# ModelCloud/GPTQModel

Hardware: NVIDIA H100
Metric: W4A16 g128 QuantLinear: decode tok/s + prefill TFLOPS vs HBM/TC roofline (higher is better)
Workload: dtype f16

## Files before the change

gptqmodel_b200/csrc/b2q_decode.cu:

```cuda
#include "b2q_common.cuh"
#include "b2q_decode.cuh"
#include "b2q_internal.h"

namespace b2q {

template <typename T, bool ASYM, bool G64, bool MOE>
__global__ void __launch_bounds__(DEC_MAX_WARPS * 32)
    decode_kernel(const __grid_constant__ DecSets S, const int32_t* __restrict__ perm, const T* __restrict__ x, int M,
                  int K, int gsh, int qpc, int max_tiles, int ngroups, int stl,
                  const __grid_constant__ DecodeAR ar, unsigned long long* __restrict__ trace) {
  using E = ET<T>;
  extern __shared__ __align__(128) uint8_t dsm[];
  auto stamp = [&](int slot) {
    if (trace != nullptr && threadIdx.x == 0 && blockIdx.y == 0) {
      unsigned long long tns;
      asm volatile("mov.u64 %0, %%globaltimer;" : "=l"(tns));
      trace[blockIdx.x * 16 + slot] = tns;
    }
  };
  stamp(0);
  if (MOE) asm volatile("griddepcontrol.wait;" ::: "memory");
  const int lane = threadIdx.x & 31, warp = threadIdx.x >> 5, nwarps = blockDim.x >> 5;
  const int g = lane >> 2, t = lane & 3;
  const int gw = nwarps / ngroups;
  const int grp = warp / gw, wg = warp - grp * gw;
  const int C = gridDim.x * ngroups;
  const int tile0 = (int)blockIdx.x * ngroups + grp;
  const int TT = S.tile_end[S.nsets - 1];
  const int ntiles = (tile0 < TT) ? (TT - tile0 + C - 1) / C : 0;
  const int nquads = K >> 7;
  const int q0 = (MOE && S.moe >= 2) ? 0 : blockIdx.y * qpc;
  const int q1 = min(q0 + qpc, nquads);
  const int kspan = qpc * 128;
  if (MOE && S.moe >= 2) x += (size_t)blockIdx.y * K * (S.moe == 3 ? 2 : 1);
  const int nst = 1 << stl;
  uint8_t* ring = dsm + (size_t)warp * nst * DEC_QUAD_BYTES;
  T* sx = reinterpret_cast<T*>(dsm + (size_t)nwarps * nst * DEC_QUAD_BYTES);
  float* xsum = reinterpret_cast<float*>(reinterpret_cast<uint8_t*>(sx) + (size_t)M * kspan * sizeof(T));
  float* red = xsum + qpc * 2 * 8;
  float* part = red + 2 * nwarps * 256;
  const uint32_t bars = smem_u32(part + max_tiles * 256) + warp * DEC_STAGES * 8;
  const bool PERM = perm != nullptr;

  const int nq = (q0 + wg < q1) ? (q1 - q0 - wg + gw - 1) / gw : 0;
  const int U = ntiles * nq;
  const uint4* iss_src = nullptr;
  size_t iss_kbs = 0;
  int iss_q = 0, iss_u = 0, iss_ti = 0;
  auto iss_begin_tile = [&]() {
    const TileRef<T> r = resolve_tile<T, MOE>(S, tile0 + iss_ti * C);
    iss_kbs = (size_t)(r.N >> 4) * 32;
    iss_src = r.w + (size_t)(2 * (q0 + wg)) * iss_kbs + (size_t)(2 * r.nt) * 32;
  };
  auto iss_one = [&](uint32_t dst, uint32_t bar) {
    issue_quad(dst, bar, iss_src, iss_kbs);
    ++iss_u;
    if (++iss_q == nq) {
      iss_q = 0;
      ++iss_ti;
      if (iss_u < U) iss_begin_tile();
    } else {
      iss_src += (size_t)(2 * gw) * iss_kbs;
    }
  };
  if (lane == 0) {
#pragma unroll
    for (int i = 0; i < DEC_STAGES; ++i) mbar_init(bars + 8 * i, 1);
    fence_mbar_init();
    if (U > 0) iss_begin_tile();
#pragma unroll
    for (int i = 0; i < DEC_STAGES; ++i)
      if (i < nst && iss_u < U) iss_one(smem_u32(ring) + i * DEC_QUAD_BYTES, bars + 8 * i);
  }
  const int gstep = (2 * gw) >> gsh;
  const int g_first = (2 * (q0 + wg)) >> gsh;
  const T* sc_next = nullptr;
  const uint32_t* zq_next = nullptr;
  int pre_q = 0, pre_ti = 0, pre_N = 0;
  auto pre_begin_tile = [&]() {
    const TileRef<T> r = resolve_tile<T, MOE>(S, tile0 + pre_ti * C);
    pre_N = r.N;
    sc_next = r.sc + (size_t)g_first * r.N + r.nt * 32 + g;
    if (ASYM) zq_next = r.zq + (size_t)g_first * (r.N >> 3) + r.nt * 4;
  };
  auto fetch_scales = [&](DScale<ASYM, G64>& d) {
#pragma unroll
    for (int i = 0; i < 4; ++i) {
      d.s[0][i] = *reinterpret_cast<const uint16_t*>(sc_next + i * 8);
      if (ASYM) d.zw[0][i] = zq_next[i];
    }
    if (G64) {
#pragma unroll
      for (int i = 0; i < 4; ++i) {
        d.s[G64 ? 1 : 0][i] = *reinterpret_cast<const uint16_t*>(sc_next + (size_t)pre_N + i * 8);
        if (ASYM) d.zw[G64 ? 1 : 0][i] = zq_next[(pre_N >> 3) + i];
      }
    }
    if (++pre_q == nq) {
      pre_q = 0;
      ++pre_ti;
      if (pre_ti < ntiles) pre_begin_tile();
    } else {
      sc_next += (size_t)gstep * pre_N;
      if (ASYM) zq_next += (size_t)gstep * (pre_N >> 3);
    }
  };
  DScale<ASYM, G64> cur;
  if (U > 0) {
    pre_begin_tile();
    fetch_scales(cur);
  }

  if (PERM) prefetch_inverse_perm(perm + K, K);
  const bool OWN = !PERM && ngroups == 1;
  if (OWN) {
    zero_own_xsum_padding(xsum, M, nq, wg, gw);
  } else {
    for (int i = threadIdx.x; i < (q1 - q0) * 2 * 8; i += blockDim.x)
      if ((i & 7) >= M) xsum[i] = 0.f;
  }
  stamp(1);
  asm volatile("griddepcontrol.launch_dependents;" ::: "memory");
  asm volatile("griddepcontrol.wait;" ::: "memory");
  stamp(2);

  if (MOE && S.moe == 3) {
    stage_x_own_quads<T, true>(x, sx, xsum, 1, K, q0, nq, wg, gw, kspan);
  } else if (OWN) {
    stage_x_own_quads<T>(x, sx, xsum, M, K, q0, nq, wg, gw, kspan);
  } else if (PERM) {
    stage_x_act_order<T>(x, perm + K, sx, xsum, M, K, q0 * 128, (q1 - q0) * 128, kspan);
  } else {
    const int n8 = (q1 - q0) * 16;
    const int tot = M * n8;
    const int totr = (tot + 31) & ~31;
    constexpr int SX_UNROLL = 4;
    auto f2 = [](uint32_t u) {
      const T* h = reinterpret_cast<const T*>(&u);
      return E::to_f(h[0]) + E::to_f(h[1]);
    };
    for (int i0 = threadIdx.x; i0 < totr; i0 += blockDim.x * SX_UNROLL) {
      uint4 xv[SX_UNROLL];
      int mm[SX_UNROLL], jj[SX_UNROLL];
#pragma unroll
      for (int u = 0; u < SX_UNROLL; ++u) {
        const int i = i0 + u * blockDim.x;
        xv[u] = make_uint4(0, 0, 0, 0);
        mm[u] = 0;
        jj[u] = 0;
        if (i < tot) {
          const int m = (M == 1) ? 0 : i / n8, j = i - m * n8;
          mm[u] = m;
          jj[u] = j;
          const T* xr = x + (size_t)m * K;
          xv[u] = reinterpret_cast<const uint4*>(xr + (size_t)q0 * 128)[j];
        }
      }
#pragma unroll
      for (int u = 0; u < SX_UNROLL; ++u) {
        const int i = i0 + u * blockDim.x;
        if (i < totr) {
          if (i < tot) reinterpret_cast<uint4*>(sx + (size_t)mm[u] * kspan)[jj[u]] = xv[u];
          float sm = (f2(xv[u].x) + f2(xv[u].y)) + (f2(xv[u].z) + f2(xv[u].w));
          sm += __shfl_xor_sync(0xffffffffu, sm, 1);
          sm += __shfl_xor_sync(0xffffffffu, sm, 2);
          sm += __shfl_xor_sync(0xffffffffu, sm, 4);
          if ((i & 7) == 0 && i < tot) xsum[(jj[u] >> 3) * 8 + mm[u]] = sm;
        }
      }
    }
  }
  if (!OWN) __syncthreads();
  stamp(3);

  constexpr float ZSYM = 8.f;
  const uint32_t nrank = cluster_nctarank();
  const uint32_t ring_a = smem_u32(ring) + lane * 16;
  const uint32_t xf_a0 = smem_u32(sx) + (uint32_t)((g * kspan + t * 16 + wg * 128) * 2);
  const uint32_t xs_a0 = smem_u32(xsum) + (uint32_t)((2 * t + wg * 16) * 4);
  const uint32_t xf_qstep = (uint32_t)gw * 256u, xs_qstep = (uint32_t)gw * 64u;
  uint32_t ar_seq = 0;
  if (ar.world > 1) ar_seq = *reinterpret_cast<const volatile uint32_t*>(ar.ctl);
  int u = 0;
  for (int ti = 0; ti < ntiles; ++ti) {
    const TileRef<T> tr = resolve_tile<T, MOE>(S, tile0 + ti * C);
    const int nt = tr.nt, N = tr.N;
    const T* bias = tr.bias;
    T* out = tr.out;
    float tot[2][4];
#pragma unroll
    for (int a = 0; a < 2; ++a)
#pragma unroll
      for (int b = 0; b < 4; ++b) tot[a][b] = 0.f;

    uint32_t xf_a = xf_a0, xs_a = xs_a0;
    for (int qi = 0; qi < nq; ++qi, ++u, xf_a += xf_qstep, xs_a += xs_qstep) {
      DScale<ASYM, G64> nxt;
      if (u + 1 < U) fetch_scales(nxt);
      const int st = u & (nst - 1);
      mbar_wait(bars + 8 * st, (uint32_t)(u >> stl) & 1u);
      const uint32_t wq_a = ring_a + st * DEC_QUAD_BYTES;
      float dd[2][2][4];
#pragma unroll
      for (int a = 0; a < 2; ++a)
#pragma unroll
        for (int b = 0; b < 2; ++b)
#pragma unroll
          for (int c = 0; c < 4; ++c) dd[a][b][c] = 0.f;
      float xs0 = 0.f, xs1 = 0.f;
#pragma unroll
      for (int kbl = 0; kbl < 2; ++kbl) {
        uint32_t bx[8];
        if (g < M) {
          const uint4 x0 = lds128(xf_a + kbl * 128), x1 = lds128(xf_a + kbl * 128 + 16);
          bx[0] = x0.x; bx[1] = x0.y; bx[2] = x0.z; bx[3] = x0.w;
          bx[4] = x1.x; bx[5] = x1.y; bx[6] = x1.z; bx[7] = x1.w;
        } else {
#pragma unroll
          for (int r = 0; r < 8; ++r) bx[r] = 0u;
        }
#pragma unroll
        for (int ftl = 0; ftl < 2; ++ftl) {
          const uint4 wv = lds128(wq_a + (kbl * 2 + ftl) * 512);
          const uint32_t w[4] = {wv.x, wv.y, wv.z, wv.w};
#pragma unroll
          for (int s = 0; s < 4; ++s) {
            uint32_t a[4];
            E::unpack_w4(w[s], a);
            mma_16816<T>(dd[kbl][ftl], a, bx[2 * s], bx[2 * s + 1]);
          }
        }
        const float2 xs = lds_f2(xs_a + kbl * 32);
        xs0 += xs.x;
        xs1 += xs.y;
        if (kbl == 1 || G64) {
          const int gi = G64 ? kbl : 0;
#pragma unroll
          for (int ftl = 0; ftl < 2; ++ftl) {
            const uint16_t slr = cur.s[gi][ftl * 2], shr = cur.s[gi][ftl * 2 + 1];
            const float sl = E::to_f(*reinterpret_cast<const T*>(&slr));
            const float sh = E::to_f(*reinterpret_cast<const T*>(&shr));
            float zl = ZSYM, zh = ZSYM;
            if (ASYM) {
              zl = (float)((cur.zw[ASYM ? gi : 0][ftl * 2] >> (4 * g)) & 15u);
              zh = (float)((cur.zw[ASYM ? gi : 0][ftl * 2 + 1] >> (4 * g)) & 15u);
            }
            const float bl = E::LO_BASE + zl, bh = E::HI_BASE + zh;
            float d[4];
#pragma unroll
            for (int c = 0; c < 4; ++c) d[c] = G64 ? dd[kbl][ftl][c] : dd[0][ftl][c] + dd[1][ftl][c];
            tot[ftl][0] = fmaf(sl, d[0] - bl * xs0, tot[ftl][0]);
            tot[ftl][1] = fmaf(sl, d[1] - bl * xs1, tot[ftl][1]);
            tot[ftl][2] = fmaf(sh, d[2] * E::HI_SCALE - bh * xs0, tot[ftl][2]);
            tot[ftl][3] = fmaf(sh, d[3] * E::HI_SCALE - bh * xs1, tot[ftl][3]);
          }
          xs0 = xs1 = 0.f;
        }
      }
      __syncwarp();
      if (lane == 0 && iss_u < U) iss_one(ring_a + st * DEC_QUAD_BYTES, bars + 8 * st);
      if (u + 1 < U) cur = nxt;
    }

    if (ti < 5) stamp(4 + 2 * ti);
    float* rbuf = red + (grp * 2 + (ti & 1)) * gw * 256;
#pragma unroll
    for (int a = 0; a < 2; ++a)
#pragma unroll
      for (int b = 0; b < 4; ++b) rbuf[(wg * 8 + a * 4 + b) * 32 + lane] = tot[a][b];
    asm volatile("bar.sync %0, %1;" ::"r"(1 + grp), "r"(gw * 32) : "memory");
    for (int i = wg * 32 + lane; i < 256; i += gw * 32) {
      float v = 0.f;
      for (int w = 0; w < gw; ++w) v += rbuf[w * 256 + i];
      if (nrank > 1) {
        part[(grp * max_tiles + ti) * 256 + i] = v;
      } else {
        const int acc = i >> 5, ln = i & 31;
        const int m = 2 * (ln & 3) + (acc & 1);
        if (m < M) {
          const int n = nt * 32 + (acc >> 2) * 16 + (ln >> 2) + ((acc & 2) ? 8 : 0);
          if (ar.world > 1) {
            if (bias != nullptr) v += E::to_f(bias[n]);
            const size_t o = ((size_t)(ar_seq & 1u) * ar.world + ar.rank) * (size_t)ar.max_elems + (size_t)m * N + n;
            for (int p = 0; p < ar.world; ++p) reinterpret_cast<float*>(ar.buf[p])[o] = v;
          } else {
            T o = E::from_f(v);
            if (bias != nullptr) o = E::from_f(E::to_f(o) + E::to_f(bias[n]));
            out[(size_t)m * N + n] = o;
          }
        }
      }
    }
    if (ti < 5) stamp(5 + 2 * ti);
  }
  stamp(15);

  if (ar.world > 1) {
    __threadfence_system();
    __syncthreads();
    const int cta = (int)blockIdx.x;
    if ((int)threadIdx.x < ar.world) {
      const int p = threadIdx.x;
      uint32_t* peer_flags = reinterpret_cast<uint32_t*>(reinterpret_cast<char*>(ar.buf[p]) + ar.flag_offset);
      asm volatile("st.release.sys.global.u32 [%0], %1;" ::"l"(peer_flags + ar.rank * 160 + cta), "r"(ar_seq + 1u)
                   : "memory");
      const uint32_t* my_flags =
          reinterpret_cast<const uint32_t*>(reinterpret_cast<const char*>(ar.buf[ar.rank]) + ar.flag_offset);
      if (!spin_until_geq_sys(my_flags + p * 160 + cta, ar_seq + 1u)) ar.ctl[2] = 1u + (uint32_t)p;
    }
    __syncthreads();
    if (ntiles > 0) {
      const TileRef<T> tr = resolve_tile<T, MOE>(S, tile0);
      const float* mine = reinterpret_cast<const float*>(ar.buf[ar.rank]) + (size_t)(ar_seq & 1u) * ar.world * ar.max_elems;
      for (int i = wg * 32 + lane; i < 256; i += gw * 32) {
        const int acc = i >> 5, ln = i & 31;
        const int m = 2 * (ln & 3) + (acc & 1);
        if (m < M) {
          const int n = tr.nt * 32 + (acc >> 2) * 16 + (ln >> 2) + ((acc & 2) ? 8 : 0);
          float v = 0.f;
          for (int p = 0; p < ar.world; ++p) v += __ldcg(mine + (size_t)p * ar.max_elems + (size_t)m * tr.N + n);
          tr.out[(size_t)m * tr.N + n] = E::from_f(v);
        }
      }
    }
    if (threadIdx.x == 0) {
      __threadfence();
      const unsigned total = gridDim.x * gridDim.y;
      if (atomicAdd(ar.ctl + 1, 1u) == total - 1u) {
        ar.ctl[1] = 0u;
        __threadfence();
        *reinterpret_cast<volatile uint32_t*>(ar.ctl) = ar_seq + 1u;
      }
    }
  }

  if (nrank > 1) {
    __syncthreads();
    cluster_sync_all();
    const uint32_t rank = cluster_ctarank();
    for (int ti = (int)rank; ti < ntiles; ti += (int)nrank) {
      const TileRef<T> tr = resolve_tile<T, MOE>(S, tile0 + ti * C);
      const int nt = tr.nt, N = tr.N;
      const T* bias = tr.bias;
      T* out = tr.out;
      for (int i = wg * 32 + lane; i < 256; i += gw * 32) {
        const int acc = i >> 5, ln = i & 31;
        const int m = 2 * (ln & 3) + (acc & 1);
        if (m < M) {
          float v = 0.f;
          for (uint32_t r = 0; r < nrank; ++r) {
            float pr = ld_dsmem_f32(smem_u32(&part[(grp * max_tiles + ti) * 256 + i]), r);
            if (MOE && S.moe >= 2) pr = S.wts[r] * E::to_f(E::from_f(pr));
            v += pr;
          }
          const int n = nt * 32 + (acc >> 2) * 16 + (ln >> 2) + ((acc & 2) ? 8 : 0);
          T o = E::from_f(v);
          if (bias != nullptr) o = E::from_f(E::to_f(o) + E::to_f(bias[n]));
          out[(size_t)m * N + n] = o;
        }
      }
    }
    cluster_sync_all();
  }
}

void* g_trace_ptr = nullptr;

struct DecodeCfg {
  int C, ks, warps, qpc, max_tiles, ngroups, stl;
  size_t smem;
};

static size_t decode_smem(int M, int warps, int qpc, int max_tiles, int nst) {
  return (size_t)warps * nst * DEC_QUAD_BYTES + (size_t)M * qpc * 128 * 2 + (size_t)qpc * 2 * 8 * 4 +
         (size_t)2 * warps * 256 * 4 + (size_t)max_tiles * 256 * 4 + (size_t)warps * DEC_STAGES * 8 + 16;
}

static bool decode_config(const MmArgs& a, int NT, DecodeCfg& best) {
  const int quads = a.K / 128;
  const int SMS = num_sms();
  double best_cost = 1e30;
  bool found = false;
  const bool two_groups = env().decode_groups2 != 0;
  for (int ks = 1; ks <= 8; ks *= 2) {
    if (a.tune_ks > 0 && ks != a.tune_ks) continue;
    if (ks > quads) break;
    const int qpc = (quads + ks - 1) / ks;
    for (int warps = 4; warps <= DEC_MAX_WARPS; warps *= 2) {
      if (a.tune_warps > 0 && warps != a.tune_warps) continue;
      int ngroups = 1;
      if (two_groups && warps == 16 && ks == 1) ngroups = 2;
      const int gwarps = warps / ngroups;
      int C = SMS / ks;
      if (C * ngroups > NT) C = (NT + ngroups - 1) / ngroups;
      if (C < 1) C = 1;
      const int max_tiles = (NT + C * ngroups - 1) / (C * ngroups);
      int stl = 2;
      size_t smem = decode_smem(a.M, warps, qpc, ks > 1 ? max_tiles * ngroups : 0, 4);
      if (smem > 200 * 1024) {
        stl = 1;
        smem = decode_smem(a.M, warps, qpc, ks > 1 ? max_tiles * ngroups : 0, 2);
      }
      if (smem > 200 * 1024) continue;
      const int qpw = (qpc + gwarps - 1) / gwarps;
      const double cost =
          (double)max_tiles * (qpw + 0.35) / ngroups + (ks > 1 ? 0.6 : 0.0) + (16 - warps) * 0.04 * max_tiles * qpw;
      if (cost < best_cost) {
        best_cost = cost;
        best = DecodeCfg{C, ks, warps, qpc, ks > 1 ? max_tiles : 0, ngroups, stl, smem};
        found = true;
      }
    }
  }
  return found;
}

bool decode2_plan(const MmArgs& a, int NT, int* out8);

bool decode_plan(int version, const MmArgs& a, int NT, int* out8) {
  if (version == 2) return decode2_plan(a, NT, out8);
  DecodeCfg c;
  if (!decode_config(a, NT, c)) return false;
  const int v[8] = {c.C, c.ks, c.warps, c.warps / c.ngroups, c.qpc, c.max_tiles, 1 << c.stl, (int)c.smem};
  for (int i = 0; i < 8; ++i) out8[i] = v[i];
  return true;
}

template <typename T, bool ASYM, bool G64, bool MOE = false>
static int launch_decode_t(const MmArgs& a, const DecSets& sets, const DecodeCfg& c, const DecodeAR& ar) {
  auto kern = decode_kernel<T, ASYM, G64, MOE>;
  if (c.smem > 48 * 1024) {
    cudaError_t e = cudaFuncSetAttribute(kern, cudaFuncAttributeMaxDynamicSharedMemorySize, (int)c.smem);
    if (e != cudaSuccess) return (int)e;
  }
  cudaLaunchConfig_t cfg = {};
  cfg.gridDim = dim3(c.C, c.ks, 1);
  cfg.blockDim = dim3(c.warps * 32, 1, 1);
  cfg.dynamicSmemBytes = c.smem;
  cfg.stream = a.stream;
  cudaLaunchAttribute attr[2];
  attr[0].id = cudaLaunchAttributeClusterDimension;
  attr[0].val.clusterDim.x = 1;
  attr[0].val.clusterDim.y = c.ks;
  attr[0].val.clusterDim.z = 1;
  attr[1].id = cudaLaunchAttributeProgrammaticStreamSerialization;
  attr[1].val.programmaticStreamSerializationAllowed = 1;
  cfg.attrs = attr;
  cfg.numAttrs = a.pdl ? 2 : 1;
  int gsh = 31;
  if (a.group_size == 64) gsh = 0;
  else if (a.group_size == 128) gsh = 1;
  cudaError_t e = cudaLaunchKernelEx(&cfg, kern, sets, a.perm, (const T*)a.x, a.M, a.K, gsh, c.qpc, c.max_tiles,
                                     c.ngroups, c.stl, ar, (unsigned long long*)g_trace_ptr);
  return (int)e;
}

bool decode_supported(const MmArgs& a) {
  return a.bits == 4 && a.M >= 1 && a.M <= DEC_MAXM && a.K % 128 == 0 && a.N % 32 == 0 &&
         (a.group_size == 64 || a.group_size == 128 || a.group_size == a.K);
}

int launch_decode2_sets(const MmArgs& a, const DecSets& sets);

static int launch_decode_sets(const MmArgs& a, const DecSets& sets) {
  {
    const int mode = env().decode_v2;
    const int NT = sets.tile_end[sets.nsets - 1];
    if (mode == 1 || (mode < 0 && NT > num_sms() && a.tune_ks <= 0 && a.tune_warps <= 0)) {
      MmArgs a2 = a;
      if (mode < 0) {
        a2.tune_ks = 1;
        a2.tune_warps = 16;
      }
      const int rc = launch_decode2_sets(a2, sets);
      if (rc != -2) return rc;
    }
  }
  DecodeCfg c;
  if (!decode_config(a, sets.tile_end[sets.nsets - 1], c)) {
    set_error("b2q_decode: no configuration fits shared memory for M=%d K=%d (ks=%d warps=%d)", a.M, a.K, a.tune_ks,
              a.tune_warps);
    return -1;
  }
  const bool asym = a.qzeros != nullptr, g64 = a.group_size == 64;
  const DecodeAR none = {};
#define B2Q_DEC_CASE(T, MOE)                                                     \
  (asym ? (g64 ? launch_decode_t<T, true, true, MOE>(a, sets, c, none)           \
               : launch_decode_t<T, true, false, MOE>(a, sets, c, none))         \
        : (g64 ? launch_decode_t<T, false, true, MOE>(a, sets, c, none)          \
               : launch_decode_t<T, false, false, MOE>(a, sets, c, none)))
  if (sets.moe != 0) return a.dtype == 0 ? B2Q_DEC_CASE(__half, true) : B2Q_DEC_CASE(__nv_bfloat16, true);
  return a.dtype == 0 ? B2Q_DEC_CASE(__half, false) : B2Q_DEC_CASE(__nv_bfloat16, false);
#undef B2Q_DEC_CASE
}

int launch_decode1_allreduce(const MmArgs& a, const DecSets& sets, const DecodeAR& ar) {
  const int NT = sets.tile_end[sets.nsets - 1];
  if (NT > num_sms() || a.perm != nullptr) return -2;
  MmArgs a1 = a;
  a1.tune_ks = 1;
  DecodeCfg c;
  if (!decode_config(a1, NT, c) || c.ks != 1 || c.ngroups != 1 || c.C < NT || c.C > 160) return -2;
  const bool asym = a.qzeros != nullptr, g64 = a.group_size == 64;
#define B2Q_DEC_CASE(T)                                                          \
  (asym ? (g64 ? launch_decode_t<T, true, true>(a1, sets, c, ar)                 \
               : launch_decode_t<T, true, false>(a1, sets, c, ar))               \
        : (g64 ? launch_decode_t<T, false, true>(a1, sets, c, ar)                \
               : launch_decode_t<T, false, false>(a1, sets, c, ar)))
  return a.dtype == 0 ? B2Q_DEC_CASE(__half) : B2Q_DEC_CASE(__nv_bfloat16);
#undef B2Q_DEC_CASE
}

int launch_decode(const MmArgs& a) {
  if (!decode_supported(a)) {
    set_error("b2q_decode: unsupported (bits=%d M=%d K=%d N=%d group=%d)", a.bits, a.M, a.K, a.N, a.group_size);
    return -1;
  }
  DecSets sets = {};
  sets.nsets = 1;
  sets.tile_end[0] = a.N / 32;
  sets.N[0] = a.N;
  sets.packed[0] = (const uint4*)a.packed;
  sets.scales[0] = a.scales;
  sets.qzeros[0] = (const uint32_t*)a.qzeros;
  sets.bias[0] = a.bias;
  sets.out[0] = a.out;
  return launch_decode_sets(a, sets);
}

int launch_decode_multi(const MmArgs& a, int nsets, const void* const* packed, const void* const* scales,
                        const int32_t* const* qzeros, const void* const* bias, void* const* out, const int* Ns) {
  if (nsets < 1 || nsets > DEC_MAX_SETS) {
    set_error("b2q_decode_multi: nsets=%d out of range (1..%d)", nsets, DEC_MAX_SETS);
    return -1;
  }
  DecSets sets = {};
  sets.nsets = nsets;
  int tiles = 0;
  for (int i = 0; i < nsets; ++i) {
    MmArgs ai = a;
    ai.N = Ns[i];
    if (!decode_supported(ai) || Ns[i] % 32 != 0 || packed[i] == nullptr || scales[i] == nullptr ||
        out[i] == nullptr || ((qzeros[i] != nullptr) != (qzeros[0] != nullptr))) {
      set_error("b2q_decode_multi: set %d unsupported (N=%d; all sets must share bits=4, K, group size and symmetry)", i,
                Ns[i]);
      return -1;
    }
    tiles += Ns[i] / 32;
    sets.tile_end[i] = tiles;
    sets.N[i] = Ns[i];
    sets.packed[i] = (const uint4*)packed[i];
    sets.scales[i] = scales[i];
    sets.qzeros[i] = (const uint32_t*)qzeros[i];
    sets.bias[i] = bias[i];
    sets.out[i] = out[i];
  }
  for (int i = nsets; i < DEC_MAX_SETS; ++i) sets.tile_end[i] = tiles;
  MmArgs a0 = a;
  a0.qzeros = qzeros[0];
  return launch_decode_sets(a0, sets);
}

static void moe_strides(DecSets& sets, int K, int N, int group_size) {
  const size_t G = (size_t)K / (size_t)group_size;
  sets.estride_w = (size_t)K * (size_t)N / 2 / 16;
  sets.estride_s = G * (size_t)N;
  sets.estride_z = G * (size_t)N / 8;
}

int launch_moe_decode_gate_up(const MmArgs& a, const void* packed1, const void* scales1, const int32_t* qzeros1,
                              const void* packed3, const void* scales3, const int32_t* qzeros3, const int32_t* ids,
                              int top_k, int E, void* gu) {
  if (!decode_supported(a) || a.M != 1 || top_k < 1 || top_k > 8 || (qzeros1 != nullptr) != (qzeros3 != nullptr)) {
    set_error("b2q_moe_decode_gate_up: needs one token, bits=4, K %% 128 == 0, group_size 64|128|K, 1 <= top_k <= 8 "
              "(M=%d K=%d N=%d g=%d top_k=%d)", a.M, a.K, a.N, a.group_size, top_k);
    return -1;
  }
  DecSets sets = {};
  sets.nsets = 1;
  const int tiles = 2 * top_k * (a.N / 32);
  for (int i = 0; i < DEC_MAX_SETS; ++i) sets.tile_end[i] = tiles;
  sets.N[0] = a.N;
  sets.packed[0] = (const uint4*)packed1;
  sets.packed[1] = (const uint4*)packed3;
  sets.scales[0] = scales1;
  sets.scales[1] = scales3;
  sets.qzeros[0] = (const uint32_t*)qzeros1;
  sets.qzeros[1] = (const uint32_t*)qzeros3;
  sets.out[0] = gu;
  sets.moe = 1;
  sets.nexperts = E;
  sets.ids = ids;
  moe_strides(sets, a.K, a.N, a.group_size);
  MmArgs a0 = a;
  a0.qzeros = qzeros1;
  a0.perm = nullptr;
  a0.bias = nullptr;
  a0.out = gu;
  return launch_decode_sets(a0, sets);
}

int launch_moe_decode_down(const MmArgs& a, const int32_t* ids, const float* wts, int top_k, int E, int fused_act) {
  if (!decode_supported(a) || a.M != 1 || !(top_k == 2 || top_k == 4 || top_k == 8)) {
    set_error("b2q_moe_decode_down: needs one token, bits=4, K %% 128 == 0, group_size 64|128|K, top_k 2|4|8 (M=%d K=%d N=%d "
              "g=%d top_k=%d)", a.M, a.K, a.N, a.group_size, top_k);
    return -1;
  }
  DecSets sets = {};
  sets.nsets = 1;
  const int NT = a.N / 32;
  for (int i = 0; i < DEC_MAX_SETS; ++i) sets.tile_end[i] = NT;
  sets.N[0] = a.N;
  sets.packed[0] = (const uint4*)a.packed;
  sets.scales[0] = a.scales;
  sets.qzeros[0] = (const uint32_t*)a.qzeros;
  sets.out[0] = a.out;
  sets.moe = fused_act ? 3 : 2;
  sets.nexperts = E;
  sets.ids = ids;
  sets.wts = wts;
  moe_strides(sets, a.K, a.N, a.group_size);
  DecodeCfg c = {};
  c.ks = top_k;
  c.warps = DEC_MAX_WARPS;
  c.ngroups = 1;
  c.qpc = a.K / 128;
  c.C = num_sms() / top_k;
  if (c.C > NT) c.C = NT;
  c.max_tiles = (NT + c.C - 1) / c.C;
  c.stl = 2;
  c.smem = decode_smem(1, c.warps, c.qpc, c.max_tiles, 4);
  if (c.smem > 200 * 1024) {
    c.stl = 1;
    c.smem = decode_smem(1, c.warps, c.qpc, c.max_tiles, 2);
  }
  if (c.smem > 200 * 1024) {
    set_error("b2q_moe_decode_down: K=%d does not fit shared memory", a.K);
    return -1;
  }
  MmArgs a0 = a;
  a0.perm = nullptr;
  a0.bias = nullptr;
  const bool asym = a.qzeros != nullptr, g64 = a.group_size == 64;
  const DecodeAR none = {};
#define B2Q_DEC_CASE(T)                                                            \
  (asym ? (g64 ? launch_decode_t<T, true, true, true>(a0, sets, c, none)           \
               : launch_decode_t<T, true, false, true>(a0, sets, c, none))         \
        : (g64 ? launch_decode_t<T, false, true, true>(a0, sets, c, none)          \
               : launch_decode_t<T, false, false, true>(a0, sets, c, none)))
  return a.dtype == 0 ? B2Q_DEC_CASE(__half) : B2Q_DEC_CASE(__nv_bfloat16);
#undef B2Q_DEC_CASE
}

}
```

gptqmodel_b200/csrc/b2q_gemm.cu:

```cuda
#include <cuda.h>

#include "b2q_common.cuh"
#include "b2q_dequant.cuh"
#include "b2q_gemm.cuh"
#include "b2q_internal.h"
#include "b2q_wgmma.cuh"

namespace b2q {

template <typename T, int BITS, bool ASYM, int STAGES>
__global__ void __launch_bounds__(G_THREADS, 1)
    gemm_kernel(const __grid_constant__ CUtensorMap tmap_x, const __grid_constant__ GemmSets S, int M, int K,
                int gshc) {
  using C = GemmCfg<BITS, STAGES>;
  using E = ET<T>;
  extern __shared__ uint8_t smem_raw[];
  const uint32_t smem_base = (smem_u32(smem_raw) + 1023u) & ~1023u;
  uint8_t* smem = smem_raw + (smem_base - smem_u32(smem_raw));

  const uint32_t sA = smem_base;
  const uint32_t sB = sA + STAGES * C::A_BYTES;
  const uint32_t sP = sB + STAGES * C::B_BYTES;
  const uint32_t sBar = sP + STAGES * C::P_BYTES;
  const uint32_t bar_full = sBar, bar_bready = sBar + 8 * STAGES, bar_empty = sBar + 16 * STAGES;

  int set = 0, tn = blockIdx.x;
  if (S.nsets > 1 && tn >= S.tn_end[0]) {
    set = (S.nsets > 2 && tn >= S.tn_end[1]) ? 2 : 1;
    tn -= S.tn_end[set - 1];
  }
  const int N = S.N[set];
  const uint4* __restrict__ packed = S.packed[set];
  const T* __restrict__ scales = reinterpret_cast<const T*>(S.scales[set]);
  const uint32_t* __restrict__ qzeros = S.qzeros[set];

  const int warp = threadIdx.x >> 5, lane = threadIdx.x & 31;
  const int NT = N >> 5;
  const int n0 = tn * G_BN, m0 = blockIdx.y * G_BM;
  const int nt0 = n0 >> 5;
  const int ntiles = min(4, NT - nt0);
  const int nkb = K / G_BK;

  if (threadIdx.x == 0) {
    prefetch_tmap(&tmap_x);
    for (int s = 0; s < STAGES; ++s) {
      mbar_init(bar_full + 8 * s, 1);
      mbar_init(bar_bready + 8 * s, G_DQ_THREADS);
      mbar_init(bar_empty + 8 * s, 1);
    }
    fence_mbar_init();
  }
  __syncthreads();

  if (warp == 8) {
    if (lane == 0) {
      const int FT = N >> 4, ft0 = n0 >> 4;
      const uint32_t pbytes4 = (uint32_t)min(8, FT - ft0) * 512u;
      const uint32_t pbytes8 = (uint32_t)ntiles * C::SUB * 512u;
      for (int kb = 0; kb < nkb; ++kb) {
        const int s = kb % STAGES;
        const uint32_t ph = (kb / STAGES) & 1;
        mbar_wait(bar_empty + 8 * s, ph ^ 1);
        const int g0 = (2 * kb) >> gshc, g1 = (2 * kb + 1) >> gshc;
        const int nrows = (g1 != g0) ? 2 : 1;
        const uint32_t sbytes = (uint32_t)min(G_BN, N - n0) * 2u, zbytes = ASYM ? sbytes / 4u : 0u;
        mbar_expect_tx(bar_full + 8 * s,
                       C::A_BYTES + (BITS == 4 ? pbytes4 + nrows * (sbytes + zbytes) : 2 * pbytes8));
        tma_load_2d(sA + s * C::A_BYTES, &tmap_x, bar_full + 8 * s, kb * G_BK, m0);
        if (BITS == 4) {
          bulk_load(sP + s * C::P_BYTES, packed + ((size_t)kb * FT + ft0) * 32, pbytes4, bar_full + 8 * s);
          for (int r = 0; r < nrows; ++r) {
            const int gr = r ? g1 : g0;
            bulk_load(sP + s * C::P_BYTES + 4096 + r * 320, scales + (size_t)gr * N + n0, sbytes, bar_full + 8 * s);
            if (ASYM)
              bulk_load(sP + s * C::P_BYTES + 4096 + r * 320 + 256, qzeros + (size_t)gr * (N >> 3) + (n0 >> 3),
                        zbytes, bar_full + 8 * s);
          }
        } else {
#pragma unroll
          for (int j = 0; j < 2; ++j)
            bulk_load(sP + s * C::P_BYTES + j * C::P_CHUNK_BYTES,
                      packed + ((size_t)(kb * 2 + j) * NT + nt0) * C::SUB * 32, pbytes8, bar_full + 8 * s);
        }
      }
    }
  } else if (warp < 4) {
    float acc[2][G_BN / 2];
#pragma unroll
    for (int mb = 0; mb < 2; ++mb)
#pragma unroll
      for (int i = 0; i < G_BN / 2; ++i) acc[mb][i] = 0.f;
    for (int kb = 0; kb < nkb; ++kb) {
      const int s = kb % STAGES;
      const uint32_t ph = (kb / STAGES) & 1;
      mbar_wait(bar_full + 8 * s, ph);
      mbar_wait(bar_bready + 8 * s, ph);
      wgmma_fence();
      const uint64_t bdesc = wgmma_desc_k_sw128(sB + s * C::B_BYTES);
      const uint64_t adesc = wgmma_desc_k_sw128(sA + s * C::A_BYTES);
#pragma unroll
      for (int k = 0; k < G_BK / 16; ++k) {
#pragma unroll
        for (int mb = 0; mb < 2; ++mb)
          Wgmma<E::FMT, G_BN>::mma(acc[mb], adesc + 512 * mb + 2 * k, bdesc + 2 * k, (kb | k) != 0 ? 1u : 0u);
      }
      wgmma_commit();
      wgmma_wait<1>();
      if (kb > 0 && threadIdx.x == 0) mbar_arrive(bar_empty + 8 * ((kb - 1) % STAGES));
    }
    wgmma_wait<0>();
#pragma unroll
    for (int mb = 0; mb < 2; ++mb) wgmma_fence_regs(acc[mb]);

    const T* __restrict__ bias = reinterpret_cast<const T*>(S.bias[set]);
    T* __restrict__ out = reinterpret_cast<T*>(S.out[set]);
#pragma unroll
    for (int mb = 0; mb < 2; ++mb) {
#pragma unroll
      for (int h = 0; h < 2; ++h) {
        const int row = m0 + 64 * mb + 16 * warp + (lane >> 2) + 8 * h;
        if (row >= M) continue;
        T* dst = out + (size_t)row * N;
#pragma unroll
        for (int j = 0; j < G_BN / 8; ++j) {
          const int col = n0 + 8 * j + 2 * (lane & 3);
          if (col >= N) continue;
          float f0 = acc[mb][4 * j + 2 * h], f1 = acc[mb][4 * j + 2 * h + 1];
          if (bias != nullptr) {
            f0 = E::to_f(E::from_f(f0)) + E::to_f(bias[col]);
            f1 = E::to_f(E::from_f(f1)) + E::to_f(bias[col + 1]);
          }
          *reinterpret_cast<uint32_t*>(dst + col) = E::pack2(f0, f1);
        }
      }
    }
  } else {
    const int t = threadIdx.x - G_MMA_THREADS;
    constexpr int PF = 32 / BITS;
    constexpr int ZSYM = 1 << (BITS - 1);
    if (BITS == 4) {
      const int lp = t & 31, g = lp >> 2, tt = lp & 3;
      int f[4];
      f[0] = (t >> 5) * 16 + g;
      f[1] = f[0] + 8;
      f[2] = f[0] + 64;
      f[3] = f[0] + 72;
      for (int kb = 0; kb < nkb; ++kb) {
        const int s = kb % STAGES;
        const uint32_t ph = (kb / STAGES) & 1;
        mbar_wait(bar_full + 8 * s, ph);
        const uint8_t* pst = smem + (sP - smem_base) + s * C::P_BYTES;
        const uint4* pj = reinterpret_cast<const uint4*>(pst);
        const int grow = ((2 * kb + (tt >> 1)) >> gshc) - ((2 * kb) >> gshc);
        const uint8_t* srow = pst + 4096 + grow * 320;
#pragma unroll
        for (int u = 0; u < 2; ++u) {
          const uint4 pv = pj[t + u * 128];
          const uint32_t s_lo = *reinterpret_cast<const uint16_t*>(srow + f[2 * u] * 2);
          const uint32_t s_hi = *reinterpret_cast<const uint16_t*>(srow + f[2 * u + 1] * 2);
          int zl = ZSYM, zh = ZSYM;
          if (ASYM) {
            const uint32_t zwl = *reinterpret_cast<const uint32_t*>(srow + 256 + (f[2 * u] >> 3) * 4);
            const uint32_t zwh = *reinterpret_cast<const uint32_t*>(srow + 256 + (f[2 * u + 1] >> 3) * 4);
            zl = (int)((zwl >> (4 * g)) & 15u);
            zh = (int)((zwh >> (4 * g)) & 15u);
          }
          uint4 lo[2], hi[2];
          Dequant<T, 4>::run(pv, s_lo, zl, s_hi, zh, lo, hi);
          const uint32_t sw = (uint32_t)g;
          const uint32_t rlo = sB + s * C::B_BYTES + f[2 * u] * 128;
          const uint32_t rhi = rlo + 8 * 128;
#pragma unroll
          for (int c = 0; c < 2; ++c) {
            const uint32_t off = (((uint32_t)(2 * tt + c)) ^ sw) << 4;
            asm volatile("st.shared.v4.u32 [%0], {%1,%2,%3,%4};" ::"r"(rlo + off), "r"(lo[c].x), "r"(lo[c].y),
                         "r"(lo[c].z), "r"(lo[c].w)
                         : "memory");
            asm volatile("st.shared.v4.u32 [%0], {%1,%2,%3,%4};" ::"r"(rhi + off), "r"(hi[c].x), "r"(hi[c].y),
                         "r"(hi[c].z), "r"(hi[c].w)
                         : "memory");
          }
        }
        fence_proxy_async_smem();
        mbar_arrive(bar_bready + 8 * s);
      }
    } else {
      const int n = n0 + t;
      const int nsafe = (n < N) ? n : 0;
      const int ntl = t >> 5;
      SZRaw cur[2], nxt[2];
      cur[0] = load_sz<T, BITS, ASYM>(scales, qzeros, 0, nsafe, N);
      cur[1] = load_sz<T, BITS, ASYM>(scales, qzeros, 1 >> gshc, nsafe, N);
      for (int kb = 0; kb < nkb; ++kb) {
        const int s = kb % STAGES;
        const uint32_t ph = (kb / STAGES) & 1;
        if (kb + 1 < nkb) {
          nxt[0] = load_sz<T, BITS, ASYM>(scales, qzeros, (2 * kb + 2) >> gshc, nsafe, N);
          nxt[1] = load_sz<T, BITS, ASYM>(scales, qzeros, (2 * kb + 3) >> gshc, nsafe, N);
        }
        mbar_wait(bar_full + 8 * s, ph);
        const uint32_t brow = sB + s * C::B_BYTES + t * 128;
        const uint32_t sw = (uint32_t)(t & 7);
#pragma unroll
        for (int j = 0; j < 2; ++j) {
          int z = ZSYM;
          if (ASYM) z = (int)((cur[j].zw >> (BITS * (nsafe % PF))) & ((1u << BITS) - 1));
          const uint4* pj = reinterpret_cast<const uint4*>(smem + (sP - smem_base) + s * C::P_BYTES +
                                                           j * C::P_CHUNK_BYTES);
#pragma unroll
          for (int h = 0; h < 2; ++h) {
            const uint4 pv = pj[(ntl * 2 + h) * 32 + lane];
            uint4 o[2];
            Dequant<T, 8>::run(pv, cur[j].s, z, o);
#pragma unroll
            for (int c = 0; c < 2; ++c) {
              const uint32_t addr = brow + (((uint32_t)(j * 4 + h * 2 + c) ^ sw) << 4);
              asm volatile("st.shared.v4.u32 [%0], {%1,%2,%3,%4};" ::"r"(addr), "r"(o[c].x), "r"(o[c].y),
                           "r"(o[c].z), "r"(o[c].w)
                           : "memory");
            }
          }
        }
        fence_proxy_async_smem();
        mbar_arrive(bar_bready + 8 * s);
        cur[0] = nxt[0];
        cur[1] = nxt[1];
      }
    }
  }
}

typedef CUresult (*EncodeTiledFn)(CUtensorMap*, CUtensorMapDataType, cuuint32_t, void*, const cuuint64_t*,
                                  const cuuint64_t*, const cuuint32_t*, const cuuint32_t*, CUtensorMapInterleave,
                                  CUtensorMapSwizzle, CUtensorMapL2promotion, CUtensorMapFloatOOBfill);

static EncodeTiledFn get_encode_fn() {
  static EncodeTiledFn fn = nullptr;
  if (fn == nullptr) {
    void* p = nullptr;
    cudaDriverEntryPointQueryResult qres;
    if (cudaGetDriverEntryPoint("cuTensorMapEncodeTiled", &p, cudaEnableDefault, &qres) == cudaSuccess &&
        qres == cudaDriverEntryPointSuccess)
      fn = reinterpret_cast<EncodeTiledFn>(p);
  }
  return fn;
}

int make_x_tmap_box(CUtensorMap* map, const void* x, int M, int K, int dtype, int box_rows) {
  struct Entry {
    const void* x;
    int M, K, dtype, box;
    CUtensorMap map;
  };
  constexpr int NCACHE = 16;
  static thread_local Entry cache[NCACHE];
  static thread_local int next = 0, filled = 0;
  for (int i = 0; i < filled; ++i) {
    const Entry& c = cache[i];
    if (c.x == x && c.M == M && c.K == K && c.dtype == dtype && c.box == box_rows) {
      *map = c.map;
      return 0;
    }
  }
  EncodeTiledFn enc = get_encode_fn();
  if (enc == nullptr) {
    set_error("b2q_gemm: cuTensorMapEncodeTiled not available from the driver");
    return -1;
  }
  cuuint64_t gdim[2] = {(cuuint64_t)K, (cuuint64_t)M};
  cuuint64_t gstride[1] = {(cuuint64_t)K * 2};
  cuuint32_t box[2] = {(cuuint32_t)G_BK, (cuuint32_t)box_rows};
  cuuint32_t estr[2] = {1, 1};
  CUresult r = enc(map, dtype == 0 ? CU_TENSOR_MAP_DATA_TYPE_FLOAT16 : CU_TENSOR_MAP_DATA_TYPE_BFLOAT16, 2,
                   const_cast<void*>(x), gdim, gstride, box, estr, CU_TENSOR_MAP_INTERLEAVE_NONE,
                   CU_TENSOR_MAP_SWIZZLE_128B, CU_TENSOR_MAP_L2_PROMOTION_L2_256B,
                   CU_TENSOR_MAP_FLOAT_OOB_FILL_NONE);
  if (r != CUDA_SUCCESS) {
    set_error("b2q_gemm: cuTensorMapEncodeTiled failed (%d) for x=%p M=%d K=%d box=%d", (int)r, x, M, K, box_rows);
    return -1;
  }
  Entry& e = cache[next];
  e.x = x;
  e.M = M;
  e.K = K;
  e.dtype = dtype;
  e.box = box_rows;
  e.map = *map;
  next = (next + 1) % NCACHE;
  if (filled < NCACHE) ++filled;
  return 0;
}

int make_x_tmap(CUtensorMap* map, const void* x, int M, int K, int dtype) {
  return make_x_tmap_box(map, x, M, K, dtype, 128);
}

int gemm_gshc(const MmArgs& a) {
  if (a.group_size == 32) return 0;
  if (a.group_size == 64) return 1;
  if (a.group_size == 128) return 2;
  return 31;
}


template <typename T, int BITS, bool ASYM, int STAGES>
static int launch_gemm_t(const MmArgs& a, const void* x, const GemmSets& S) {
  using C = GemmCfg<BITS, STAGES>;
  CUtensorMap tmap;
  if (make_x_tmap(&tmap, x, a.M, a.K, a.dtype) != 0) return -1;
  auto kern = gemm_kernel<T, BITS, ASYM, STAGES>;
  static uint32_t smem_ok = 0;
  if (int e = ensure_dyn_smem(kern, C::SMEM_BYTES, smem_ok, "b2q_gemm")) return e;
  dim3 grid(S.tn_end[S.nsets - 1], (a.M + G_BM - 1) / G_BM, 1);
  kern<<<grid, G_THREADS, C::SMEM_BYTES, a.stream>>>(tmap, S, a.M, a.K, gemm_gshc(a));
  return (int)cudaGetLastError();
}

static int launch_gemm_sets(const MmArgs& a, const void* x, const GemmSets& S) {
  const bool asym = S.qzeros[0] != nullptr;
#define B2Q_GEMM_CASE(T, BITS, ST) \
  (asym ? launch_gemm_t<T, BITS, true, ST>(a, x, S) : launch_gemm_t<T, BITS, false, ST>(a, x, S))
  if (a.dtype == 0) return a.bits == 4 ? B2Q_GEMM_CASE(__half, 4, 4) : B2Q_GEMM_CASE(__half, 8, 4);
  return a.bits == 4 ? B2Q_GEMM_CASE(__nv_bfloat16, 4, 4) : B2Q_GEMM_CASE(__nv_bfloat16, 8, 4);
#undef B2Q_GEMM_CASE
}

int launch_gemm_multi(const MmArgs& a, const void* x, int nsets, const void* const* packed, const void* const* scales,
                      const int32_t* const* qzeros, const void* const* bias, void* const* out, const int* Ns) {
  if (nsets < 1 || nsets > G_MAX_SETS) {
    set_error("b2q_gemm_multi: nsets=%d out of range (1..%d)", nsets, G_MAX_SETS);
    return -1;
  }
  if (a.K % G_BK != 0) {
    set_error("b2q_gemm_multi: K=%d must be a multiple of %d", a.K, G_BK);
    return -1;
  }
  GemmSets S = {};
  S.nsets = nsets;
  int tn = 0;
  for (int i = 0; i < nsets; ++i) {
    if (Ns[i] <= 0 || Ns[i] % 32 != 0 || packed[i] == nullptr || scales[i] == nullptr || out[i] == nullptr ||
        ((qzeros[i] != nullptr) != (qzeros[0] != nullptr))) {
      set_error("b2q_gemm_multi: set %d unsupported (N=%d; all sets share K, group size and symmetry)", i, Ns[i]);
      return -1;
    }
    tn += (Ns[i] + G_BN - 1) / G_BN;
    S.tn_end[i] = tn;
    S.N[i] = Ns[i];
    S.packed[i] = (const uint4*)packed[i];
    S.scales[i] = scales[i];
    S.qzeros[i] = (const uint32_t*)qzeros[i];
    S.bias[i] = bias[i];
    S.out[i] = out[i];
  }
  for (int i = nsets; i < G_MAX_SETS; ++i) S.tn_end[i] = tn;
  return launch_gemm_sets(a, x, S);
}

int launch_gemm(const MmArgs& a) {
  if (a.K % G_BK != 0) {
    set_error("b2q_gemm: K=%d must be a multiple of %d", a.K, G_BK);
    return -1;
  }
  const void* x = a.x;
  if (a.perm != nullptr) {
    const size_t need = (size_t)a.M * a.K * 2;
    if (a.workspace == nullptr || a.workspace_bytes < need) {
      set_error("b2q_gemm: act-order needs a %zu-byte workspace (got %zu)", need, a.workspace_bytes);
      return -1;
    }
    int e = launch_permute_cols(a.x, a.perm, a.workspace, a.M, a.K, a.stream);
    if (e != 0) return e;
    x = a.workspace;
  }
  if (a.M <= 128 && env().midm && midm_supported(a)) return launch_midm(a, x);
  const void* packed = a.packed;
  const void* scales = a.scales;
  const int32_t* qzeros = (const int32_t*)a.qzeros;
  const void* bias = a.bias;
  void* out = a.out;
  return launch_gemm_multi(a, x, 1, &packed, &scales, &qzeros, &bias, &out, &a.N);
}

}
```

gptqmodel_b200/csrc/b2q_gemm.cuh:

```cuda
#pragma once
#include "b2q_common.cuh"

namespace b2q {

constexpr int G_BM = 128;
constexpr int G_BN = 128;
constexpr int G_BK = 64;
constexpr int G_MMA_THREADS = 128;
constexpr int G_DQ_THREADS = 128;
constexpr int G_THREADS = G_MMA_THREADS + G_DQ_THREADS + 32;

template <int BITS, int STAGES>
struct GemmCfg {
  static constexpr int SUB = BITS / 4;
  static constexpr int A_BYTES = G_BM * G_BK * 2;
  static constexpr int B_BYTES = G_BN * G_BK * 2;
  static constexpr int P_CHUNK_BYTES = 4 * SUB * 512;
  static constexpr int P_BYTES = 2 * P_CHUNK_BYTES + (BITS == 4 ? 1024 : 0);
  static constexpr int STAGE_BYTES = A_BYTES + B_BYTES + P_BYTES;
  static constexpr int BAR_BYTES = 256;
  static constexpr int SMEM_BYTES = STAGES * STAGE_BYTES + BAR_BYTES + 1024;
  static_assert(SMEM_BYTES <= 227 * 1024, "dynamic shared memory of one CTA");
};

constexpr int G_MAX_SETS = 3;
struct GemmSets {
  int nsets;
  int tn_end[G_MAX_SETS];
  int N[G_MAX_SETS];
  const uint4* packed[G_MAX_SETS];
  const void* scales[G_MAX_SETS];
  const uint32_t* qzeros[G_MAX_SETS];
  const void* bias[G_MAX_SETS];
  void* out[G_MAX_SETS];
};

}
```

Before: 585.5.

## Add two-consumer-warpgroup GEMM variant with register reallocation and decode v2 routing

The prefill GEMM kernel is templated on the number of consumer warpgroups. With two consumers, each CTA covers 256 rows of M and reuses one dequantized B tile across both, which halves the dequant work per output. Warpgroup roles now set their register budgets with setmaxnreg, and a wave-count heuristic picks between one and two consumers. Separately, the decode path now routes non-MoE calls to the v2 decode kernel even when there are fewer tiles than SMs. The trade-off is more shared memory per CTA and possible tail or occupancy problems when M is small.

```diff
diff --git a/gptqmodel_b200/csrc/b2q_decode.cu b/gptqmodel_b200/csrc/b2q_decode.cu
--- a/gptqmodel_b200/csrc/b2q_decode.cu
+++ b/gptqmodel_b200/csrc/b2q_decode.cu
@@ -466,9 +466,9 @@
   {
     const int mode = env().decode_v2;
     const int NT = sets.tile_end[sets.nsets - 1];
-    if (mode == 1 || (mode < 0 && NT > num_sms() && a.tune_ks <= 0 && a.tune_warps <= 0)) {
+    if (mode == 1 || (mode < 0 && a.tune_ks <= 0 && a.tune_warps <= 0 && (NT > num_sms() || sets.moe == 0))) {
       MmArgs a2 = a;
-      if (mode < 0) {
+      if (mode < 0 && NT > num_sms()) {
         a2.tune_ks = 1;
         a2.tune_warps = 16;
       }
diff --git a/gptqmodel_b200/csrc/b2q_gemm.cu b/gptqmodel_b200/csrc/b2q_gemm.cu
--- a/gptqmodel_b200/csrc/b2q_gemm.cu
+++ b/gptqmodel_b200/csrc/b2q_gemm.cu
@@ -8,11 +8,21 @@
 
 namespace b2q {
 
-template <typename T, int BITS, bool ASYM, int STAGES>
-__global__ void __launch_bounds__(G_THREADS, 1)
+template <int REGS>
+__device__ __forceinline__ void setmaxnreg_inc() {
+  asm volatile("setmaxnreg.inc.sync.aligned.u32 %0;" ::"n"(REGS));
+}
+template <int REGS>
+__device__ __forceinline__ void setmaxnreg_dec() {
+  asm volatile("setmaxnreg.dec.sync.aligned.u32 %0;" ::"n"(REGS));
+}
+
+template <typename T, int BITS, bool ASYM, int STAGES, int CWG>
+__global__ void __launch_bounds__(GemmRoles<CWG>::THREADS, 1)
     gemm_kernel(const __grid_constant__ CUtensorMap tmap_x, const __grid_constant__ GemmSets S, int M, int K,
                 int gshc) {
-  using C = GemmCfg<BITS, STAGES>;
+  using C = GemmCfg<BITS, STAGES, CWG>;
+  using R = GemmRoles<CWG>;
   using E = ET<T>;
   extern __shared__ uint8_t smem_raw[];
   const uint32_t smem_base = (smem_u32(smem_raw) + 1023u) & ~1023u;
@@ -34,9 +44,9 @@
   const T* __restrict__ scales = reinterpret_cast<const T*>(S.scales[set]);
   const uint32_t* __restrict__ qzeros = S.qzeros[set];
 
-  const int warp = threadIdx.x >> 5, lane = threadIdx.x & 31;
+  const int wg = threadIdx.x / G_WG, warp = (threadIdx.x >> 5) & 3, lane = threadIdx.x & 31;
   const int NT = N >> 5;
-  const int n0 = tn * G_BN, m0 = blockIdx.y * G_BM;
+  const int n0 = tn * G_BN, m0 = blockIdx.y * R::BM;
   const int nt0 = n0 >> 5;
   const int ntiles = min(4, NT - nt0);
   const int nkb = K / G_BK;
@@ -45,15 +55,16 @@
     prefetch_tmap(&tmap_x);
     for (int s = 0; s < STAGES; ++s) {
       mbar_init(bar_full + 8 * s, 1);
-      mbar_init(bar_bready + 8 * s, G_DQ_THREADS);
-      mbar_init(bar_empty + 8 * s, 1);
+      mbar_init(bar_bready + 8 * s, G_WG);
+      mbar_init(bar_empty + 8 * s, CWG);
     }
     fence_mbar_init();
   }
   __syncthreads();
 
-  if (warp == 8) {
-    if (lane == 0) {
+  if (wg == CWG + 1) {
+    setmaxnreg_dec<R::PRODUCER_REGS>();
+    if (warp == 0 && lane == 0) {
       const int FT = N >> 4, ft0 = n0 >> 4;
       const uint32_t pbytes4 = (uint32_t)min(8, FT - ft0) * 512u;
       const uint32_t pbytes8 = (uint32_t)ntiles * C::SUB * 512u;
@@ -84,7 +95,8 @@
         }
       }
     }
-  } else if (warp < 4) {
+  } else if (wg < CWG) {
+    setmaxnreg_inc<R::CONSUMER_REGS>();
     float acc[2][G_BN / 2];
 #pragma unroll
     for (int mb = 0; mb < 2; ++mb)
@@ -97,7 +109,7 @@
       mbar_wait(bar_bready + 8 * s, ph);
       wgmma_fence();
       const uint64_t bdesc = wgmma_desc_k_sw128(sB + s * C::B_BYTES);
-      const uint64_t adesc = wgmma_desc_k_sw128(sA + s * C::A_BYTES);
+      const uint64_t adesc = wgmma_desc_k_sw128(sA + s * C::A_BYTES + wg * (G_BM * G_BK * 2));
 #pragma unroll
       for (int k = 0; k < G_BK / 16; ++k) {
 #pragma unroll
@@ -106,7 +118,7 @@
       }
       wgmma_commit();
       wgmma_wait<1>();
-      if (kb > 0 && threadIdx.x == 0) mbar_arrive(bar_empty + 8 * ((kb - 1) % STAGES));
+      if (kb > 0 && threadIdx.x % G_WG == 0) mbar_arrive(bar_empty + 8 * ((kb - 1) % STAGES));
     }
     wgmma_wait<0>();
 #pragma unroll
@@ -118,7 +130,7 @@
     for (int mb = 0; mb < 2; ++mb) {
 #pragma unroll
       for (int h = 0; h < 2; ++h) {
-        const int row = m0 + 64 * mb + 16 * warp + (lane >> 2) + 8 * h;
+        const int row = m0 + G_BM * wg + 64 * mb + 16 * warp + (lane >> 2) + 8 * h;
         if (row >= M) continue;
         T* dst = out + (size_t)row * N;
 #pragma unroll
@@ -135,7 +147,8 @@
       }
     }
   } else {
-    const int t = threadIdx.x - G_MMA_THREADS;
+    setmaxnreg_dec<R::DEQUANT_REGS>();
+    const int t = threadIdx.x - CWG * G_WG;
     constexpr int PF = 32 / BITS;
     constexpr int ZSYM = 1 << (BITS - 1);
     if (BITS == 4) {
@@ -291,10 +304,6 @@
   return 0;
 }
 
-int make_x_tmap(CUtensorMap* map, const void* x, int M, int K, int dtype) {
-  return make_x_tmap_box(map, x, M, K, dtype, 128);
-}
-
 int gemm_gshc(const MmArgs& a) {
   if (a.group_size == 32) return 0;
   if (a.group_size == 64) return 1;
@@ -303,17 +312,27 @@
 }
 
 
+template <typename T, int BITS, bool ASYM, int STAGES, int CWG>
+static int launch_gemm_cwg(const MmArgs& a, const void* x, const GemmSets& S) {
+  using C = GemmCfg<BITS, STAGES, CWG>;
+  using R = GemmRoles<CWG>;
+  CUtensorMap tmap;
+  if (make_x_tmap_box(&tmap, x, a.M, a.K, a.dtype, R::BM) != 0) return -1;
+  auto kern = gemm_kernel<T, BITS, ASYM, STAGES, CWG>;
+  static uint32_t smem_ok = 0;
+  if (int e = ensure_dyn_smem(kern, C::SMEM_BYTES, smem_ok, "b2q_gemm")) return e;
+  dim3 grid(S.tn_end[S.nsets - 1], (a.M + R::BM - 1) / R::BM, 1);
+  kern<<<grid, R::THREADS, C::SMEM_BYTES, a.stream>>>(tmap, S, a.M, a.K, gemm_gshc(a));
+  return (int)cudaGetLastError();
+}
+
 template <typename T, int BITS, bool ASYM, int STAGES>
 static int launch_gemm_t(const MmArgs& a, const void* x, const GemmSets& S) {
-  using C = GemmCfg<BITS, STAGES>;
-  CUtensorMap tmap;
-  if (make_x_tmap(&tmap, x, a.M, a.K, a.dtype) != 0) return -1;
-  auto kern = gemm_kernel<T, BITS, ASYM, STAGES>;
-  static uint32_t smem_ok = 0;
-  if (int e = ensure_dyn_smem(kern, C::SMEM_BYTES, smem_ok, "b2q_gemm")) return e;
-  dim3 grid(S.tn_end[S.nsets - 1], (a.M + G_BM - 1) / G_BM, 1);
-  kern<<<grid, G_THREADS, C::SMEM_BYTES, a.stream>>>(tmap, S, a.M, a.K, gemm_gshc(a));
-  return (int)cudaGetLastError();
+  const long ncols = S.tn_end[S.nsets - 1], sms = num_sms();
+  const long waves1 = (ncols * ((a.M + GemmRoles<1>::BM - 1) / GemmRoles<1>::BM) + sms - 1) / sms;
+  const long waves2 = (ncols * ((a.M + GemmRoles<2>::BM - 1) / GemmRoles<2>::BM) + sms - 1) / sms;
+  if (3 * waves2 < 2 * waves1) return launch_gemm_cwg<T, BITS, ASYM, STAGES, 2>(a, x, S);
+  return launch_gemm_cwg<T, BITS, ASYM, STAGES, 1>(a, x, S);
 }
 
 static int launch_gemm_sets(const MmArgs& a, const void* x, const GemmSets& S) {
diff --git a/gptqmodel_b200/csrc/b2q_gemm.cuh b/gptqmodel_b200/csrc/b2q_gemm.cuh
--- a/gptqmodel_b200/csrc/b2q_gemm.cuh
+++ b/gptqmodel_b200/csrc/b2q_gemm.cuh
@@ -6,14 +6,24 @@
 constexpr int G_BM = 128;
 constexpr int G_BN = 128;
 constexpr int G_BK = 64;
-constexpr int G_MMA_THREADS = 128;
-constexpr int G_DQ_THREADS = 128;
-constexpr int G_THREADS = G_MMA_THREADS + G_DQ_THREADS + 32;
+constexpr int G_WG = 128;
 
-template <int BITS, int STAGES>
+template <int CWG>
+struct GemmRoles {
+  static constexpr int THREADS = (CWG + 2) * G_WG;
+  static constexpr int BM = CWG * G_BM;
+  static constexpr int CONSUMER_REGS = 176;
+  static constexpr int DEQUANT_REGS = 120;
+  static constexpr int PRODUCER_REGS = 40;
+  static_assert(BM <= 256, "TMA box height");
+  static_assert(CWG * CONSUMER_REGS + DEQUANT_REGS + PRODUCER_REGS <= (65536 / THREADS / 8 * 8) * (CWG + 2),
+                "setmaxnreg budget of one CTA");
+};
+
+template <int BITS, int STAGES, int CWG>
 struct GemmCfg {
   static constexpr int SUB = BITS / 4;
-  static constexpr int A_BYTES = G_BM * G_BK * 2;
+  static constexpr int A_BYTES = CWG * G_BM * G_BK * 2;
   static constexpr int B_BYTES = G_BN * G_BK * 2;
   static constexpr int P_CHUNK_BYTES = 4 * SUB * 512;
   static constexpr int P_BYTES = 2 * P_CHUNK_BYTES + (BITS == 4 ? 1024 : 0);
```

After: 624.9 (median of 6 runs). +6.7%, better.
